# Bergvca/string_grouper

Hardware: AMD Instinct MI355X
Metric: hot-path rows/sec (the device path of match_strings: tokenise + tf-idf + postings + SpGEMM-topn, inputs resident in HBM), 663k-name self-join ntop=10 min_sim=0.8; match_strings end to end: match_strings_rows_per_s (higher is better)
Workload: dtype f32

## Files before the change

### string_grouper_amd/csrc/sg_collapse.hip

```cpp
#include <cstddef>
#include <memory>

#include "sg_internal.h"
#include "sg_scan.h"

template <typename T>
__global__ void __launch_bounds__(256) row_hash_kernel(const int64_t *__restrict__ indptr, const int32_t *__restrict__ indices,
                                                       const T *__restrict__ data, int64_t n_rows, uint64_t *__restrict__ hash,
                                                       uint32_t *__restrict__ row_id ) {
    const int64_t r = ((int64_t)blockIdx.x * blockDim.x + threadIdx.x) >> 4;
    const int sub = threadIdx.x & 15;
    uint64_t h = 0;
    if (r < n_rows) {
        const int64_t lo = indptr[r], hi = indptr[r + 1];
        for (int64_t p = lo + sub; p < hi; p += 16) {
            uint64_t v;
            if (sizeof(T) == 4) v = (uint64_t)__float_as_uint((float)data[p]);
            else v = (uint64_t)__double_as_longlong((double)data[p]);
            uint64_t x = ((uint64_t)(uint32_t)indices[p] << 32) ^ v ^ ((uint64_t)(p - lo) * 0x9E3779B97F4A7C15ull);
            x ^= x >> 33;
            x *= 0xff51afd7ed558ccdull;
            x ^= x >> 33;
            x *= 0xc4ceb9fe1a85ec53ull;
            x ^= x >> 33;
// ... 578 lines not shown
    return SG_OK;
}

struct SortWork {
    uint64_t *hash = nullptr, *hash_sorted = nullptr;
    uint32_t *row_id = nullptr, *row_sorted = nullptr, *head = nullptr, *run_excl = nullptr, *head_pos = nullptr;
    uint32_t *rep_of_row = nullptr, *rank_of_row = nullptr, *is_rep = nullptr, *rep_excl = nullptr, *size = nullptr;
    uint32_t *totals = nullptr;
};

static int sort_and_count(Scratch &scratch, const sg_csr *B, SortWork *w, uint32_t *n_groups) {
    sg_ctx *ctx = scratch.ctx;
    const int64_t n = B->n_rows;
    const unsigned g1 = (unsigned)((n + 255) / 256), g16 = (unsigned)((n * 16 + 255) / 256);
    SG_TRY(scratch.alloc((size_t)n + 1, &w->hash));
    SG_TRY(scratch.alloc((size_t)40, &w->totals));
    SG_TRY(scratch.alloc((size_t)n + 1, &w->hash_sorted));
    SG_TRY(scratch.alloc((size_t)n + 1, &w->row_id));
    SG_TRY(scratch.alloc((size_t)n + 1, &w->row_sorted));
    SG_TRY(scratch.alloc((size_t)n + 1, &w->head));
    SG_TRY(scratch.alloc((size_t)n + 1, &w->run_excl));
    by_dtype(B->dtype, [&](auto tag) {
        using T = decltype(tag);
        hipLaunchKernelGGL(row_hash_kernel<T>, dim3(g16), dim3(256), 0, ctx->stream, B->d_indptr, B->d_indices, (const T *)B->d_data, n,
                           w->hash, w->row_id);
        return SG_OK;
    });
    SG_TRY(sg_sort_pairs_u64_u32(ctx, w->hash, w->row_id, n, w->hash_sorted, w->row_sorted));
    by_dtype(B->dtype, [&](auto tag) {
        using T = decltype(tag);
        hipLaunchKernelGGL(group_heads_kernel<T>, dim3(g1), dim3(256), 0, ctx->stream, B->d_indptr, B->d_indices, (const T *)B->d_data, n,
                           (const uint64_t *)w->hash_sorted, (const uint32_t *)w->row_sorted, w->head);
        return SG_OK;
    });
    SG_TRY(sg_exclusive_scan_u32(ctx, w->head, w->run_excl, n, w->totals));
    SG_HIP_TRY(hipMemcpyAsync(n_groups, w->totals, 4, hipMemcpyDeviceToHost, ctx->stream));
    SG_HIP_TRY(hipStreamSynchronize(ctx->stream));
    return SG_OK;
}

static int sorted_members(Scratch &scratch, int64_t n, SortWork *w, SgCollapse *c) {
    sg_ctx *ctx = scratch.ctx;
    const int64_t n_u = c->n_u;
    const unsigned g1 = (unsigned)((n + 255) / 256);
    SG_TRY(scratch.alloc((size_t)n_u + 1, &w->size));
    SG_TRY(sg_alloc(ctx, (size_t)n + 1, &c->d_gid));
    SG_TRY(sg_alloc(ctx, (size_t)n_u + 2, &c->d_group_ptr));
    SG_TRY(sg_alloc(ctx, (size_t)n + 1, &c->d_members));
    SG_TRY(sg_alloc(ctx, (size_t)n_u + 1, &c->d_rep_rows));
    SG_TRY(scratch.alloc((size_t)n_u + 1, &w->head_pos));
    SG_TRY(scratch.alloc((size_t)n + 1, &w->rep_of_row));
    SG_TRY(scratch.alloc((size_t)n + 1, &w->rank_of_row));
    SG_TRY(scratch.alloc((size_t)n + 1, &w->is_rep));
    SG_TRY(scratch.alloc((size_t)n + 1, &w->rep_excl));
    SG_TRY(SG_ZERO2(ctx, w->is_rep, sizeof(uint32_t) * (size_t)(n + 1), w->size, sizeof(uint32_t) * (size_t)(n_u + 1)));
    hipLaunchKernelGGL(head_pos_kernel, dim3(g1), dim3(256), 0, ctx->stream, (const uint32_t *)w->head, (const uint32_t *)w->run_excl, n,
                       w->head_pos);
    hipLaunchKernelGGL(group_members_kernel, dim3(g1), dim3(256), 0, ctx->stream, (const uint32_t *)w->head,
                       (const uint32_t *)w->run_excl, (const uint32_t *)w->head_pos, (const uint32_t *)w->row_sorted, n, w->rep_of_row,
                       w->rank_of_row, w->is_rep);
    SG_TRY(sg_exclusive_scan_u32(ctx, w->is_rep, w->rep_excl, n, nullptr));
    hipLaunchKernelGGL(group_ids_kernel, dim3(g1), dim3(256), 0, ctx->stream, (const uint32_t *)w->rep_of_row,
                       (const uint32_t *)w->rep_excl, (const uint32_t *)w->is_rep, n, c->d_gid, w->size, c->d_rep_rows,
                       (const int64_t *)nullptr, (int64_t *)nullptr, (int32_t *)nullptr, (unsigned long long *)nullptr);
    SG_TRY(sg_exclusive_scan_u32(ctx, w->size, c->d_group_ptr, n_u, c->d_group_ptr + n_u));
    hipLaunchKernelGGL(group_fill_kernel, dim3(g1), dim3(256), 0, ctx->stream, (const uint32_t *)c->d_gid,
                       (const uint32_t *)w->rank_of_row, (const uint32_t *)c->d_group_ptr, n, c->d_members);
    SG_HIP_TRY(hipGetLastError());
    return SG_OK;
}

static int unique_row_pointers(Scratch &scratch, const sg_csr *B, const SgCollapse *c, int64_t **ptr, int64_t *nnz_u) {
    sg_ctx *ctx = scratch.ctx;
    const int64_t n_u = c->n_u;
    int32_t *len = nullptr;
    SG_TRY(scratch.alloc((size_t)n_u + 1, &len));
    SG_TRY(scratch.alloc((size_t)n_u + 2, ptr));
    hipLaunchKernelGGL(unique_len_kernel, dim3((unsigned)((n_u + 255) / 256)), dim3(256), 0, ctx->stream, B->d_indptr,
                       (const uint32_t *)c->d_rep_rows, n_u, len);
    SG_TRY(sg_exclusive_scan_i32_to_i64(ctx, len, *ptr, n_u));
    SG_HIP_TRY(hipMemcpyAsync(nnz_u, *ptr + n_u, 8, hipMemcpyDeviceToHost, ctx->stream));
    SG_HIP_TRY(hipStreamSynchronize(ctx->stream));
    scratch.keep(*ptr);
    return SG_OK;
}

static int group_by_sort(sg_ctx *ctx, const sg_csr *B, bool forced, bool defer_rows, SgCollapse **out) {
    *out = nullptr;
    const int64_t n = B->n_rows;
    CollapsePtr c;
    int64_t *ptr = nullptr;
    int64_t nnz_u = 0;
    {
        Scratch scratch(ctx);
        SortWork w;
        uint32_t n_groups = 0;
        SG_TRY(sort_and_count(scratch, B, &w, &n_groups));
        if (!worth_grouping(n_groups, n, forced)) return SG_OK;
        c = new_groups(ctx, n);
        if (!c) return SG_ERR_OOM;
        c->n_u = n_groups;
        SG_TRY(sorted_members(scratch, n, &w, c.get()));
        SG_TRY(unique_row_pointers(scratch, B, c.get(), &ptr, &nnz_u));
    }
    SG_TRY(collapse_unique_matrix(ctx, B, c.get(), nnz_u, ptr, defer_rows));
    *out = c.release();
    return SG_OK;
}

int sg_collapse_build(sg_ctx *ctx, const sg_csr *B, SgCollapse **out, bool left_side, bool defer_rows) {
    *out = nullptr;
    bool forced = false;
    if (!wanted(ctx, B, left_side, &forced)) return SG_OK;
    bool by_sort = ctx->opt_is("SG_GROUP_SORT", '1');
    if (!by_sort) SG_TRY(group_by_hash_table(ctx, B, forced, defer_rows, out, &by_sort));
    if (by_sort) SG_TRY(group_by_sort(ctx, B, forced, defer_rows, out));
    return SG_OK;
}

template <typename T>
__global__ void __launch_bounds__(256) expand_simple_kernel(const int32_t *__restrict__ u_cols, const T *__restrict__ u_vals,
                                                            const int32_t *__restrict__ u_cnt, int32_t u_stride,
                                                            const uint32_t *__restrict__ gid ,
                                                            const int32_t *__restrict__ row_list ,
                                                            const uint32_t *__restrict__ group_ptr, const uint32_t *__restrict__ members,
                                                            int64_t n_out, int32_t stride, int32_t *__restrict__ cols,
                                                            T *__restrict__ vals, int32_t *__restrict__ cnt,
                                                            uint32_t *__restrict__ slow_count, uint32_t *__restrict__ slow_rows) {
    const int64_t r = (int64_t)blockIdx.x * blockDim.x + threadIdx.x;
    if (r >= n_out) return;
    const int64_t row = row_list ? (int64_t)row_list[r] : r;
    const int64_t ur = gid ? (int64_t)gid[row] : row;
    const int32_t m = u_cnt[ur];
    const int32_t *uc = u_cols + ur * u_stride;
    const T *uv = u_vals + ur * u_stride;
    int32_t out = 0;
    T prev = (T)0;
    for (int32_t e = 0; e < m && out < stride; ++e) {
        const uint32_t lo = group_ptr[uc[e]], hi = group_ptr[uc[e] + 1];
        const T v = uv[e];
        if (hi - lo != 1u && ((e > 0 && prev == v) || (e + 1 < m && uv[e + 1] == v))) {
            slow_rows[atomicAdd(slow_count, 1u)] = (uint32_t)r;
            return;
        }
        for (uint32_t p = lo; p < hi && out < stride; ++p, ++out) {
            cols[r * stride + out] = (int32_t)members[p];
            vals[r * stride + out] = v;
        }
        prev = v;
    }
    cnt[r] = out;
}

template <typename T>
__global__ void __launch_bounds__(64) expand_merge_kernel(const int32_t *__restrict__ u_cols, const T *__restrict__ u_vals,
                                                          const int32_t *__restrict__ u_cnt, int32_t u_stride,
                                                          const uint32_t *__restrict__ gid, const int32_t *__restrict__ row_list,
                                                          const uint32_t *__restrict__ group_ptr,
                                                          const uint32_t *__restrict__ members, int32_t stride,
                                                          int32_t *__restrict__ cols, T *__restrict__ vals, int32_t *__restrict__ cnt,
                                                          const uint32_t *__restrict__ slow_count, const uint32_t *__restrict__ slow_rows) {
    const int lane = threadIdx.x;
    const uint32_t n_slow = *slow_count;
    for (uint32_t q = blockIdx.x; q < n_slow; q += gridDim.x) {
        const int64_t r = slow_rows[q];
        const int64_t row = row_list ? (int64_t)row_list[r] : r;
        const int64_t ur = gid ? (int64_t)gid[row] : row;
        const int32_t m = u_cnt[ur];
        const int32_t *uc = u_cols + ur * u_stride;
        const T *uv = u_vals + ur * u_stride;
        int32_t out = 0;
        int32_t e0 = 0;
        while (e0 < m && out < stride) {
            const T score = uv[e0];
            int32_t e1 = e0 + 1;
            while (e1 < m && uv[e1] == score) ++e1;
            const int32_t run = e1 - e0;
            if (run <= 64) {
                uint32_t cur = 0, end = 0;
                if (lane < run) {
                    cur = group_ptr[uc[e0 + lane]];
                    end = group_ptr[uc[e0 + lane] + 1];
                }
                uint32_t nxt = (lane < run && cur < end) ? members[cur] : 0xFFFFFFFFu;
                while (out < stride) {
                    uint32_t best = nxt;
#pragma unroll
                    for (int d = 32; d > 0; d >>= 1) best = min(best, (uint32_t)__shfl_xor((int)best, d, 64));
                    if (best == 0xFFFFFFFFu) break;
                    if (lane == 0) {
                        cols[r * stride + out] = (int32_t)best;
                        vals[r * stride + out] = score;
                    }
                    ++out;
                    if (nxt == best) {
                        ++cur;
                        nxt = cur < end ? members[cur] : 0xFFFFFFFFu;
                    }
                }
            } else {
                uint32_t last = 0;
                bool any_written = false;
                while (out < stride) {
                    uint32_t best = 0xFFFFFFFFu;
                    for (int32_t g = lane; g < run; g += 64) {
                        uint32_t lo = group_ptr[uc[e0 + g]], hi = group_ptr[uc[e0 + g] + 1];
                        while (lo < hi) {
                            const uint32_t mid = (lo + hi) >> 1;
                            if (any_written && members[mid] <= last) lo = mid + 1;
                            else hi = mid;
                        }
                        if (lo < group_ptr[uc[e0 + g] + 1]) best = min(best, members[lo]);
                    }
#pragma unroll
                    for (int d = 32; d > 0; d >>= 1) best = min(best, (uint32_t)__shfl_xor((int)best, d, 64));
                    if (best == 0xFFFFFFFFu) break;
                    if (lane == 0) {
                        cols[r * stride + out] = (int32_t)best;
                        vals[r * stride + out] = score;
                    }
                    ++out;
                    last = best;
                    any_written = true;
                }
            }
            e0 = e1;
        }
        if (lane == 0) cnt[r] = out;
    }
}

int sg_collapse_expand(sg_ctx *ctx, const SgCollapse *c, const sg_topn *ru, bool rows_are_groups, sg_topn *out,
                       const int32_t *row_list) {
    const int64_t n_out = out->n_rows;
    if (n_out <= 0) return SG_OK;
    Scratch scratch(ctx);
    uint32_t *slow = nullptr;
    SG_TRY(scratch.alloc((size_t)n_out + 4, &slow));
    SG_TRY(SG_ZERO2(ctx, out->d_counts, sizeof(int32_t) * (size_t)(n_out + 1), slow, 16));
    const unsigned g1 = (unsigned)((n_out + 255) / 256);
    const uint32_t *gid = rows_are_groups ? c->d_gid : nullptr;
    by_dtype(out->dtype, [&](auto tag) {
        using T = decltype(tag);
        hipLaunchKernelGGL(expand_simple_kernel<T>, dim3(g1), dim3(256), 0, ctx->stream, (const int32_t *)ru->d_cols,
                           (const T *)ru->d_vals, (const int32_t *)ru->d_counts, ru->stride, gid, row_list,
                           (const uint32_t *)c->d_group_ptr, (const uint32_t *)c->d_members, n_out, out->stride, out->d_cols,
                           (T *)out->d_vals, out->d_counts, slow, slow + 4);
        hipLaunchKernelGGL(expand_merge_kernel<T>, dim3(2048), dim3(64), 0, ctx->stream, (const int32_t *)ru->d_cols,
                           (const T *)ru->d_vals, (const int32_t *)ru->d_counts, ru->stride, gid, row_list,
                           (const uint32_t *)c->d_group_ptr, (const uint32_t *)c->d_members, out->stride, out->d_cols,
                           (T *)out->d_vals, out->d_counts, (const uint32_t *)slow, (const uint32_t *)(slow + 4));
        return SG_OK;
    });
    SG_HIP_TRY(hipGetLastError());
    return SG_OK;
}
```

### string_grouper_amd/csrc/sg_spgemm_topn.hip

```cpp
#include <cstring>
#include <math.h>

#include <memory>

#include "sg_internal.h"

#include "sg_k4_device.h"
#include "sg_plan.h"

static_assert(SG_PLAN_LANES == SG_TOPN_LANES, "sg_plan.h counts passes and register lists in the kernels' lanes");

typedef float f32x4 __attribute__((ext_vector_type(4)));
typedef double f64x2 __attribute__((ext_vector_type(2)));
template <typename T, typename V>
__device__ __forceinline__ bool any_above(const V &v, T thr);
template <>
__device__ __forceinline__ bool any_above<float, f32x4>(const f32x4 &v, float thr) {
    const uint32_t a = __float_as_uint(v[0]), b = __float_as_uint(v[1]), c = __float_as_uint(v[2]),
                   d = __float_as_uint(v[3]);
    const uint32_t ab = a > b ? a : b, cd = c > d ? c : d;
    return (ab > cd ? ab : cd) > __float_as_uint(thr);
}
template <>
__device__ __forceinline__ bool any_above<double, f64x2>(const f64x2 &v, double thr) {
// ... 559 lines not shown
    a->nnz = A->nnz;
    a->f64 = A->dtype == SG_F64;
    a->is_index_source = built_from(A, Bt);
    b->cosine_like = Bt->cosine_like;
    b->has_filter = Bt->d_filt != nullptr;
    b->tile_form = Bt->tile_form;
    b->pruned_tile = sg_pruned_supports_tile(Bt->tile_log2);
    b->fold_log2 = Bt->fold_log2;
    b->tile_log2 = Bt->tile_log2;
    b->n_tiles = Bt->n_tiles;
    b->n_right = Bt->n_right;
    b->nnz = Bt->nnz;
    b->n_terms = Bt->n_terms;
    const sg_csr *from = companion_source(A, Bt);
    b->source_rows = from ? from->n_rows : -1;
}

static int plan_multiply(sg_ctx *ctx, const sg_csr *A, const sg_postings *Bt, int32_t top_n, double threshold, bool row_range,
                         SgPlan *plan) {
    *plan = SgPlan();
    const SgPlanSwitches sw = multiply_switches(ctx);
    SgPlanCall call;
    call.threshold = plan->threshold = sg_plan_clamp_threshold(threshold);
    call.row_range = row_range;
    plan->index = Bt;
    if (!result_stride(A->n_rows, top_n, Bt->n_right, &plan->stride))
        return row_range ? SG_OK : result_overflow(A->n_rows, plan->stride, "; split the left matrix");
    call.stride = plan->stride;
    SgPlanLeft a;
    SgPlanIndex b;
    describe(A, Bt, &a, &b);

    if (sg_plan_wants_tile_form(a, b, call, sw) && sg_plan_source_fits(b)) {
        SG_TRY(companion(ctx, owner(Bt), SgCompanion::alt_tile, companion_source(A, Bt), &Bt));
        describe(A, Bt, &a, &b);
    }

    bool a_cosine_like = false;
    if (sg_plan_needs_props(a, b, call, sw)) {
        plan->delta = sg_plan_delta(a, b, call, sw);
        float a_n2 = 0.f;
        SG_TRY(sg_csr_props(ctx, A, &a_cosine_like, &a_n2, nullptr));
    }

    plan->form = sg_plan_form(a, b, call, sw, a_cosine_like);

    if (sg_plan_pilot_due(a, b, call, sw, plan->form)) {
        SgPilotPrices prices;
        SG_TRY(sg_csr_ensure_rows(ctx, A));
        SG_TRY(prune_pilot(ctx, A, Bt, a, b, plan->stride, plan->threshold, plan->delta, plan->form == SgPlan::PRUNED_SELFJOIN, &prices));
        plan->form = sg_plan_after_pilot(plan->form, prices, sw);
    }

    const SgOwnIndex own = sg_plan_exact_own_index(a, b, call, sw, plan->form);
    if (own != SgOwnIndex::none) {
        SG_TRY(companion(ctx, owner(Bt), SgCompanion::exact_native, own == SgOwnIndex::from_left ? A : companion_source(A, Bt), &Bt));
        describe(A, Bt, &a, &b);
    }

    plan->index = Bt;
    plan->launch = sg_plan_launch_shape(a, b, plan->stride, ctx->num_cu, ctx->lds_per_cu, sw);
    return SG_OK;
}

static int zero_then_selfjoin_pass(sg_ctx *ctx, const sg_csr *A, const SgPlan &plan, sg_topn *r, uint32_t *counters, size_t n_counters,
                                   size_t n_stat_words, bool *done, int64_t row_lo = 0, int64_t row_hi = -1,
                                   int32_t **d_pairs = nullptr, int64_t *n_pairs = nullptr, int64_t row_step = 1) {
    *done = false;
    SG_TRY(SG_ZERO3(ctx, counters, sizeof(uint32_t) * n_counters, r->d_counts, sizeof(int32_t) * (size_t)A->n_rows,
                    ctx->d_stat_words, n_stat_words * sizeof(int64_t)));
    int st = SG_OK;
    if (sg_plan_selfjoin(plan.form))
        st = sg_spgemm_pruned_symmetric(ctx, A, plan.index, plan.stride, r, plan.threshold, plan.delta,
                                        (unsigned long long *)(ctx->d_stat_words + 2), done, row_lo, row_hi, d_pairs, n_pairs, row_step,
                                        plan.form == SgPlan::EXACT_SELFJOIN);
    ctx->prune_symmetric = *done;
    return st;
}

static int pruned_launches(sg_ctx *ctx, const sg_csr *A, const SgPlan &plan, sg_topn *r, uint32_t *row_counter, uint32_t *handed_count,
                           uint32_t *handed_rows) {
    SgTimer kt(ctx, SG_K_SPGEMM_KERNEL);
    SG_TRY(sg_spgemm_pruned_launch(ctx, A, plan.index, plan.stride < SG_TOPN_LANES ? plan.stride : SG_TOPN_LANES, r, plan.threshold,
                                   plan.delta, row_counter, handed_count, handed_rows, (unsigned long long *)(ctx->d_stat_words + 2)));
    if (plan.stride > SG_TOPN_LANES && A->n_rows > 0) {
        hipLaunchKernelGGL(rows_with_full_lists_kernel, dim3((unsigned)((A->n_rows + 255) / 256)), dim3(256), 0, ctx->stream,
                           (const int32_t *)r->d_counts, A->n_rows, (int32_t)SG_TOPN_LANES, handed_count, handed_rows);
        SG_HIP_TRY(hipGetLastError());
    }
    return SG_OK;
}

static int rows_handed_over(sg_ctx *ctx, const sg_postings *Bt, const uint32_t *handed_count, bool *any) {
    *any = true;
    if (Bt->d_vals != nullptr || Bt->nnz <= 0) return SG_OK;
    uint32_t *h_handed = (uint32_t *)(ctx->h_stat_words + 7);
    *h_handed = 0;
    SG_TRY(sg_fetch(ctx, h_handed, handed_count, 4));
    *any = *h_handed > 0;
    return SG_OK;
}

static int exact_passes(sg_ctx *ctx, const sg_csr *A, const SgPlan &plan, sg_topn *r, uint32_t *counters, const uint32_t *row_list,
                        const uint32_t *row_list_len) {
    const sg_postings *Bt = plan.index;
    const SgLaunchShape &sh = plan.launch;
    if (A->n_rows <= 0) return SG_OK;
    for (int pass = 0, li = 0; pass < sh.n_pass; ++pass) {
        const int pass_off = pass * SG_TOPN_LANES;
        const int keep = plan.stride - pass_off < SG_TOPN_LANES ? plan.stride - pass_off : SG_TOPN_LANES;
        for (int g = 0; g < sh.n_groups; ++g, ++li) {
            const int tb = g * sh.group;
            const int te = tb + sh.group < Bt->n_tiles ? tb + sh.group : Bt->n_tiles;
            SG_TRY(by_dtype(A->dtype, [&](auto tag) {
                using T = decltype(tag);
                return dispatch_spgemm<T>(ctx, A, Bt, tb, te, keep, pass_off, r, (T)plan.threshold, counters + li, sh.grid, row_list, row_list_len);
            }));
        }
    }
    return SG_OK;
}

static int run_plan(sg_ctx *ctx, const sg_csr *A, const SgPlan &plan, sg_topn *r) {
    const sg_postings *Bt = plan.index;
    const bool prune = sg_plan_pruned(plan.form);
    const size_t n_launch = (size_t)plan.launch.n_launch(), n_words = n_launch + 4;
    Scratch tmp(ctx);
    uint32_t *counters = nullptr;
    SG_TRY(tmp.alloc(n_words + (prune ? (size_t)A->n_rows : 0), &counters));
    uint32_t *handed_count = counters + n_launch + 2;
    uint32_t *handed_rows = counters + n_words;

    SgTimer timer(ctx, SG_K_SPGEMM);
    bool selfjoin_done = false;
    SG_TRY(zero_then_selfjoin_pass(ctx, A, plan, r, counters, n_words, 7, &selfjoin_done));
    if (selfjoin_done) return SG_OK;
    SG_TRY(sg_csr_ensure_rows(ctx, A));
    if (!prune) {
        SG_TRY(sg_postings_ensure_full(ctx, Bt));
        SgTimer kt(ctx, SG_K_SPGEMM_KERNEL);
        return exact_passes(ctx, A, plan, r, counters, nullptr, handed_count);
    }
    SG_TRY(pruned_launches(ctx, A, plan, r, counters + n_launch + 1, handed_count, handed_rows));
    bool any_handed = false;
    SG_TRY(rows_handed_over(ctx, Bt, handed_count, &any_handed));
    if (any_handed) {
        SG_TRY(sg_postings_ensure_full(ctx, Bt));
        SG_TRY(exact_passes(ctx, A, plan, r, counters, handed_rows, handed_count));
    }
    SG_HIP_TRY(hipMemcpyAsync(ctx->d_stat_words + 5, handed_count, 4, hipMemcpyDeviceToDevice, ctx->stream));
    return SG_OK;
}

struct InnerMultiply {
    sg_ctx *ctx;
    explicit InnerMultiply(sg_ctx *c) : ctx(c) { ++ctx->inner_multiply_depth; }
    ~InnerMultiply() { --ctx->inner_multiply_depth; }
};

static int spgemm_topn_collapsed(sg_ctx *ctx, const sg_csr *A, const sg_postings *Bt, int32_t top_n, double threshold,
                                 int32_t sort, sg_topn **out) {
    const SgCollapse *c = Bt->collapse;
    int64_t stride64 = top_n;
    if (stride64 > c->n_orig) stride64 = c->n_orig > 0 ? c->n_orig : 1;
    if (stride64 > 2 * SG_TOPN_LANES) {
        const sg_postings *plain = nullptr;
        SG_TRY(companion(ctx, Bt, SgCompanion::plain, &Bt->caller_b_copy, &plain));
        return sg_spgemm_topn(ctx, A, plain, top_n, threshold, sort, out);
    }
    const bool self = built_from(A, Bt);
    sg_postings view = *Bt;
    view.collapse = nullptr;
    view.plain = nullptr;
    view.view_of = Bt;
    sg_topn *groups = nullptr;
    {
        const InnerMultiply inner(ctx);
        SG_TRY(sg_spgemm_topn(ctx, self ? c->unique : A, &view, top_n, threshold, 1, &groups));
    }
    const TopnPtr ru(groups);
    TopnPtr r;
    SG_TRY(topn_alloc(ctx, A->n_rows, c->n_orig, (int32_t)stride64, A->dtype, &r));
    {
        SgTimer timer(ctx, SG_K_ZIP);
        SG_TRY(sg_collapse_expand(ctx, c, ru.get(), self, r.get()));
        if (!sort) SG_TRY(sort_rows_by_column(ctx, r.get()));
        if (A->n_rows > 0 && ctx->inner_multiply_depth == 0) {
            hipLaunchKernelGGL(sum_counts_kernel, dim3(256), dim3(256), 0, ctx->stream, r->d_counts, A->n_rows,
                               (unsigned long long *)(ctx->d_stat_words + 1));
            if (hipGetLastError() != hipSuccess) return SG_ERR_HIP;
        }
    }
    *out = r.release();
    return SG_OK;
}

template <typename T>
__global__ void __launch_bounds__(256) expand_left_rows_kernel(const int32_t *__restrict__ u_cols, const T *__restrict__ u_vals,
                                                               const int32_t *__restrict__ u_cnt, const uint32_t *__restrict__ gid,
                                                               int64_t n_rows, int32_t stride, int32_t *__restrict__ cols,
                                                               T *__restrict__ vals, int32_t *__restrict__ cnt) {
    const int64_t cell = (int64_t)blockIdx.x * blockDim.x + threadIdx.x;
    if (cell >= n_rows * stride) return;
    const int64_t r = cell / stride;
    const int32_t e = (int32_t)(cell - r * stride);
    const int64_t g = gid[r];
    const int32_t m = u_cnt[g];
    if (e == 0) cnt[r] = m;
    if (e < m) {
        cols[cell] = u_cols[g * stride + e];
        vals[cell] = u_vals[g * stride + e];
    }
}

static int spgemm_topn_left_groups(sg_ctx *ctx, const sg_csr *A, const sg_postings *Bt, int32_t top_n, double threshold, int32_t sort,
                                   sg_topn **out, bool *done) {
    *done = false;
    if (A->left_state == 1) return SG_OK;
    if (A->left_state == 0) {
        SgCollapse *g = nullptr;
        bool cl = false;
        float n2 = 0.f;
        SG_TRY(sg_csr_props(ctx, A, &cl, &n2));
        if (cl) SG_TRY(sg_collapse_build(ctx, A, &g, true));
        A->left_groups = g;
        A->left_state = g ? 2 : 1;
        if (!g) return SG_OK;
    }
    const SgCollapse *g = A->left_groups;
    sg_topn *groups = nullptr;
    g->unique->left_state = 1;
    {
        const InnerMultiply inner(ctx);
        SG_TRY(sg_spgemm_topn(ctx, g->unique, Bt, top_n, threshold, sort, &groups));
    }
    const TopnPtr ru(groups);
    TopnPtr r;
    SG_TRY(topn_alloc(ctx, A->n_rows, ru->n_cols, ru->stride, ru->dtype, &r));
    if (A->n_rows > 0) {
        SgTimer timer(ctx, SG_K_ZIP);
        const int64_t cells = A->n_rows * (int64_t)ru->stride;
        const unsigned grid = (unsigned)((cells + 255) / 256);
        by_dtype(ru->dtype, [&](auto tag) {
            using T = decltype(tag);
            hipLaunchKernelGGL(expand_left_rows_kernel<T>, dim3(grid), dim3(256), 0, ctx->stream, (const int32_t *)ru->d_cols,
                               (const T *)ru->d_vals, (const int32_t *)ru->d_counts, (const uint32_t *)g->d_gid, A->n_rows,
                               ru->stride, r->d_cols, (T *)r->d_vals, r->d_counts);
            return SG_OK;
        });
        hipLaunchKernelGGL(sum_counts_kernel, dim3(256), dim3(256), 0, ctx->stream, r->d_counts, A->n_rows,
                           (unsigned long long *)(ctx->d_stat_words + 1));
        if (hipGetLastError() != hipSuccess) return SG_ERR_HIP;
    }
    *out = r.release();
    *done = true;
    return SG_OK;
}

static int left_groups_apply(sg_ctx *ctx, const sg_csr *A, const sg_postings *Bt, int32_t top_n, bool *apply) {
    *apply = false;
    const bool off = ctx->opt_is("SG_COLLAPSE", '0') || ctx->opt_is("SG_COLLAPSE_LEFT", '0');
    if (off && A->left_groups) {
        sg_collapse_free(A->left_groups);
        A->left_groups = nullptr;
        A->left_state = 0;
    }
    if (built_from(A, Bt) || off || A->left_state == 1 || A->n_cols != Bt->n_terms || A->dtype != Bt->dtype || top_n < 1) return SG_OK;
    int32_t stride = 0;
    if (!result_stride(A->n_rows, top_n, Bt->collapse ? Bt->collapse->n_orig : Bt->n_right, &stride))
        return result_overflow(A->n_rows, stride, "; split the left matrix");
    *apply = true;
    return SG_OK;
}

extern "C" int sg_spgemm_topn(sg_ctx *ctx, const sg_csr *A, const sg_postings *Bt, int32_t top_n, double threshold,
                              int32_t sort, sg_topn **out) {
    SG_REQUIRE(ctx && A && Bt && out, "null argument");
    bool group_left = false;
    SG_TRY(left_groups_apply(ctx, A, Bt, top_n, &group_left));
    if (group_left) {
        bool done = false;
        SG_TRY(spgemm_topn_left_groups(ctx, A, Bt, top_n, threshold, sort, out, &done));
        if (done) return SG_OK;
    }
    if (Bt->collapse) {
        SG_REQUIRE(A->n_cols == Bt->n_terms && A->dtype == Bt->dtype && top_n >= 1, "A and B differ in columns or value type, or top_n < 1");
        return spgemm_topn_collapsed(ctx, A, Bt, top_n, threshold, sort, out);
    }
    SG_REQUIRE(A->n_cols == Bt->n_terms, "A and B have different numbers of columns (vocabulary size)");
    SG_REQUIRE(A->dtype == Bt->dtype, "A and B have different value types");
    SG_REQUIRE(top_n >= 1, "top_n must be >= 1");
    SgPlan plan;
    SG_TRY(plan_multiply(ctx, A, Bt, top_n, threshold, false, &plan));
    Bt = plan.index;
    TopnPtr r;
    SG_TRY(topn_alloc(ctx, A->n_rows, Bt->n_right, plan.stride, A->dtype, &r));
    SG_TRY(run_plan(ctx, A, plan, r.get()));
    if (!sort) SG_TRY(sort_rows_by_column(ctx, r.get()));
    if (A->nnz > 0 && built_from(A, Bt))
        hipLaunchKernelGGL(count_macs_selfjoin_kernel, dim3(64), dim3(256), 0, ctx->stream, (const uint32_t *)Bt->d_term_len,
                           Bt->n_terms, (unsigned long long *)ctx->d_stat_words);
    else if (A->nnz > 0)
        hipLaunchKernelGGL(count_macs_kernel, dim3(512), dim3(256), 0, ctx->stream, A->d_indptr, A->d_indices,
                           A->n_rows, (const uint32_t *)Bt->d_term_len, (unsigned long long *)ctx->d_stat_words);
    if (A->n_rows > 0 && ctx->inner_multiply_depth == 0)
        hipLaunchKernelGGL(sum_counts_kernel, dim3(256), dim3(256), 0, ctx->stream, r->d_counts, A->n_rows,
                           (unsigned long long *)(ctx->d_stat_words + 1));
    record_bytes(ctx, A, Bt, plan.threshold);
    if (hipGetLastError() != hipSuccess) return SG_ERR_HIP;
    *out = r.release();
    return SG_OK;
}

extern "C" int sg_selfjoin_range(sg_ctx *ctx, const sg_csr *A, const sg_postings *Bt, int32_t top_n, double threshold,
                                 int64_t row_lo, int64_t row_hi, sg_topn **out, int32_t **d_pairs, int64_t *n_pairs,
                                 int32_t *pair_words, int32_t *applicable, int64_t row_step) {
    if (row_step < 1) row_step = 1;
    SG_REQUIRE(ctx && A && Bt && out && d_pairs && n_pairs && pair_words && applicable, "null argument");
    SG_REQUIRE(A->n_cols == Bt->n_terms && A->dtype == Bt->dtype, "A and B differ in columns or value type");
    SG_REQUIRE(top_n >= 1, "top_n must be >= 1");
    SG_REQUIRE(row_lo >= 0 && row_lo <= row_hi && row_hi <= A->n_rows, "row range outside the matrix");
    *out = nullptr;
    *d_pairs = nullptr;
    *n_pairs = 0;
    *pair_words = A->dtype == SG_F64 ? 4 : 3;
    *applicable = 0;
    if (Bt->collapse) {
        const SgCollapse *c = Bt->collapse;
        if (!built_from(A, Bt)) return SG_OK;
        if (row_hi > c->n_u) {
            sg_set_error("row range [%lld, %lld) outside the %lld groups of the index (sg_postings_rows)", (long long)row_lo,
                         (long long)row_hi, (long long)c->n_u);
            return SG_ERR_BADARG;
        }
        sg_postings view = *Bt;
        view.collapse = nullptr;
        view.plain = nullptr;
        const int st_u = sg_selfjoin_range(ctx, c->unique, &view, top_n, threshold, row_lo, row_hi, out, d_pairs, n_pairs, pair_words,
                                           applicable, row_step);
        if (st_u == SG_OK && *out) (*out)->top_n_asked = top_n;
// ... 191 lines not shown
```

Measured before the change: 111.6 million.

## Expand collapsed top-n rows with DPP sub-wave kernel and fused count sum

Replaces the one-thread-per-row expansion of collapsed group results with a kernel that assigns a 4/8/16-lane sub-wave to each row. It uses DPP row moves for tie detection and for prefix sums of group sizes, so members are scattered in parallel, and it processes several rows per thread to raise memory-level parallelism. The kernel and the merge kernel also accumulate the total result count, which removes the separate sum_counts launch. The grid becomes persistent, capped at twice the CU count. The new paths add complexity, a device-side atomic per block, and an optional probe path that synchronises the stream.

Result: no change. 111.1 million (-0.4%).

```diff
diff --git a/string_grouper_amd/csrc/sg_collapse.hip b/string_grouper_amd/csrc/sg_collapse.hip
--- a/string_grouper_amd/csrc/sg_collapse.hip
+++ b/string_grouper_amd/csrc/sg_collapse.hip
@@ -754,6 +754,163 @@
     cnt[r] = out;
 }
 
+template <int CTRL>
+__device__ __forceinline__ uint32_t row_move(uint32_t x) {
+    return (uint32_t)__builtin_amdgcn_update_dpp(0, (int)x, CTRL, 0xf, 0xf, true);
+}
+template <int CTRL>
+__device__ __forceinline__ float row_move(float x) {
+    return __uint_as_float(row_move<CTRL>(__float_as_uint(x)));
+}
+template <int CTRL>
+__device__ __forceinline__ double row_move(double x) {
+    const uint64_t b = (uint64_t)__double_as_longlong(x);
+    const uint64_t m = ((uint64_t)row_move<CTRL>((uint32_t)(b >> 32)) << 32) | row_move<CTRL>((uint32_t)b);
+    return __longlong_as_double((long long)m);
+}
+
+template <typename T, int W>
+__device__ __forceinline__ void subwave_trip(int sl, int first, int32_t e, int32_t m, T v, T below_edge, T above_edge, uint32_t lo,
+                                             uint32_t hi, uint32_t out, int32_t stride, uint32_t &at, uint32_t &n, uint32_t &total,
+                                             bool &queued) {
+    const bool has = e < m;
+    const uint32_t size = hi - lo;
+    T below = row_move<0x111>(v), above = row_move<0x101>(v);
+    if (sl == 0) below = below_edge;
+    if (sl == W - 1) above = above_edge;
+    const bool tie = has && size != 1u && ((e > 0 && below == v) || (e + 1 < m && above == v));
+    uint32_t incl = size, t;
+    t = row_move<0x111>(incl); if (sl >= 1) incl += t;
+    t = row_move<0x112>(incl); if (sl >= 2) incl += t;
+    if (W >= 8) { t = row_move<0x114>(incl); if (sl >= 4) incl += t; }
+    if (W >= 16) { t = row_move<0x118>(incl); if (sl >= 8) incl += t; }
+    total = size;
+    total += row_move<0xB1>(total);
+    total += row_move<0x4E>(total);
+    if (W >= 8) total += row_move<0x141>(total);
+    if (W >= 16) total += row_move<0x140>(total);
+    at = out + (incl - size);
+    const unsigned long long ties = __ballot(tie && at < (uint32_t)stride);
+    queued = ((ties >> first) & ((1ull << W) - 1ull)) != 0;
+    n = 0;
+    if (has && !queued && at < (uint32_t)stride) n = size < (uint32_t)stride - at ? size : (uint32_t)stride - at;
+}
+
+#define SG_EXPAND_BLOCK 512
+template <typename T, int W, int R>
+__global__ void __launch_bounds__(SG_EXPAND_BLOCK) expand_subwave_kernel(const int32_t *__restrict__ u_cols, const T *__restrict__ u_vals,
+                                                             const int32_t *__restrict__ u_cnt, int32_t u_stride,
+                                                             const uint32_t *__restrict__ gid, const int32_t *__restrict__ row_list,
+                                                             const uint32_t *__restrict__ group_ptr, const uint32_t *__restrict__ members,
+                                                             int64_t n_out, int32_t stride, int32_t *__restrict__ cols,
+                                                             T *__restrict__ vals, int32_t *__restrict__ cnt,
+                                                             uint32_t *__restrict__ slow_count, uint32_t *__restrict__ slow_rows,
+                                                             unsigned long long *__restrict__ sum_out) {
+    static_assert(W == 4 || W == 8 || W == 16, "a sub-wave is a quad, half a DPP row or a whole one");
+    const int sl = threadIdx.x & (W - 1);
+    const int first = threadIdx.x & 63 & ~(W - 1);
+    const int64_t n_sub = (int64_t)gridDim.x * blockDim.x / W;
+    uint32_t written = 0;
+    for (int64_t r0 = ((int64_t)blockIdx.x * blockDim.x + threadIdx.x) / W; r0 < n_out; r0 += n_sub * R) {
+        int64_t ur[R];
+        int32_t m[R], g[R];
+        T v[R], v_edge[R];
+        uint32_t lo[R], hi[R], at[R], n[R], out[R], member0[R];
+        bool queued[R];
+#pragma unroll
+        for (int k = 0; k < R; ++k) {
+            const int64_t r = r0 + k * n_sub;
+            ur[k] = -1;
+            if (r < n_out) {
+                const int64_t row = row_list ? (int64_t)row_list[r] : r;
+                ur[k] = gid ? (int64_t)gid[row] : row;
+            }
+        }
+#pragma unroll
+        for (int k = 0; k < R; ++k) {
+            m[k] = 0, g[k] = 0, v[k] = (T)0, v_edge[k] = (T)0;
+            if (ur[k] >= 0) {
+                m[k] = u_cnt[ur[k]];
+                if (sl < u_stride) g[k] = u_cols[ur[k] * u_stride + sl], v[k] = u_vals[ur[k] * u_stride + sl];
+                if (sl == W - 1 && W < u_stride) v_edge[k] = u_vals[ur[k] * u_stride + W];
+            }
+        }
+#pragma unroll
+        for (int k = 0; k < R; ++k) {
+            lo[k] = hi[k] = 0;
+            if (sl < m[k]) lo[k] = group_ptr[g[k]], hi[k] = group_ptr[g[k] + 1];
+        }
+#pragma unroll
+        for (int k = 0; k < R; ++k) {
+            subwave_trip<T, W>(sl, first, sl, m[k], v[k], (T)0, v_edge[k], lo[k], hi[k], 0u, stride, at[k], n[k], out[k], queued[k]);
+            member0[k] = n[k] ? members[lo[k]] : 0u;
+        }
+#pragma unroll
+        for (int k = 0; k < R; ++k) {
+            const int64_t r = r0 + k * n_sub;
+            if (n[k]) {
+                cols[r * stride + at[k]] = (int32_t)member0[k];
+                vals[r * stride + at[k]] = v[k];
+                for (uint32_t j = 1; j < n[k]; ++j) {
+                    cols[r * stride + at[k] + j] = (int32_t)members[lo[k] + j];
+                    vals[r * stride + at[k] + j] = v[k];
+                }
+            }
+        }
+#pragma unroll
+        for (int k = 0; k < R; ++k) {
+            if (ur[k] < 0) continue;
+            const int64_t r = r0 + k * n_sub;
+            const int32_t *uc = u_cols + ur[k] * u_stride;
+            const T *uv = u_vals + ur[k] * u_stride;
+            uint32_t o = out[k];
+            bool q = queued[k];
+            for (int32_t base = W; !q && base < m[k] && o < (uint32_t)stride; base += W) {
+                const int32_t e = base + sl;
+                const bool has = e < m[k];
+                const int32_t ge = has ? uc[e] : 0;
+                const T ve = has ? uv[e] : (T)0;
+                const T below_edge = (has && sl == 0) ? uv[e - 1] : (T)0;
+                const T above_edge = (sl == W - 1 && e + 1 < m[k]) ? uv[e + 1] : (T)0;
+                uint32_t l = 0, h = 0, a, c, total;
+                if (has) l = group_ptr[ge], h = group_ptr[ge + 1];
+                subwave_trip<T, W>(sl, first, e, m[k], ve, below_edge, above_edge, l, h, o, stride, a, c, total, q);
+                for (uint32_t j = 0; j < c; ++j) {
+                    cols[r * stride + a + j] = (int32_t)members[l + j];
+                    vals[r * stride + a + j] = ve;
+                }
+                o += total;
+            }
+            if (o > (uint32_t)stride) o = (uint32_t)stride;
+            if (sl == 0) {
+                if (q) {
+                    slow_rows[atomicAdd(slow_count, 1u)] = (uint32_t)r;
+                } else {
+                    cnt[r] = (int32_t)o;
+                    written += o;
+                }
+            }
+        }
+    }
+    if (sum_out) {
+        __shared__ uint32_t wave_sum[SG_EXPAND_BLOCK / 64];
+        uint32_t s = written;
+        s += row_move<0xB1>(s);
+        s += row_move<0x4E>(s);
+        s += row_move<0x141>(s);
+        s += row_move<0x140>(s);
+        const uint32_t wave = (uint32_t)__builtin_amdgcn_readlane((int)s, 0) + (uint32_t)__builtin_amdgcn_readlane((int)s, 16) +
+                              (uint32_t)__builtin_amdgcn_readlane((int)s, 32) + (uint32_t)__builtin_amdgcn_readlane((int)s, 48);
+        if ((threadIdx.x & 63) == 0) wave_sum[threadIdx.x >> 6] = wave;
+        __syncthreads();
+        if (threadIdx.x == 0) {
+            unsigned long long block = 0;
+            for (unsigned w = 0; w < blockDim.x / 64; ++w) block += wave_sum[w];
+            if (block) atomicAdd(sum_out, block);
+        }
+    }
+}
+
 template <typename T>
 __global__ void __launch_bounds__(64) expand_merge_kernel(const int32_t *__restrict__ u_cols, const T *__restrict__ u_vals,
                                                           const int32_t *__restrict__ u_cnt, int32_t u_stride,
@@ -761,7 +918,8 @@
                                                           const uint32_t *__restrict__ group_ptr,
                                                           const uint32_t *__restrict__ members, int32_t stride,
                                                           int32_t *__restrict__ cols, T *__restrict__ vals, int32_t *__restrict__ cnt,
-                                                          const uint32_t *__restrict__ slow_count, const uint32_t *__restrict__ slow_rows) {
+                                                          const uint32_t *__restrict__ slow_count, const uint32_t *__restrict__ slow_rows,
+                                                          unsigned long long *__restrict__ sum_out ) {
     const int lane = threadIdx.x;
     const uint32_t n_slow = *slow_count;
     for (uint32_t q = blockIdx.x; q < n_slow; q += gridDim.x) {
@@ -828,32 +986,62 @@
             }
             e0 = e1;
         }
-        if (lane == 0) cnt[r] = out;
-    }
-}
-
-int sg_collapse_expand(sg_ctx *ctx, const SgCollapse *c, const sg_topn *ru, bool rows_are_groups, sg_topn *out,
-                       const int32_t *row_list) {
+        if (lane == 0) {
+            cnt[r] = out;
+            if (sum_out && out) atomicAdd(sum_out, (unsigned long long)out);
+        }
+    }
+}
+
+int sg_collapse_expand_counted(sg_ctx *ctx, const SgCollapse *c, const sg_topn *ru, bool rows_are_groups, sg_topn *out,
+                               const int32_t *row_list, unsigned long long *sum_out, bool *summed) {
+    if (summed) *summed = false;
     const int64_t n_out = out->n_rows;
     if (n_out <= 0) return SG_OK;
     Scratch scratch(ctx);
     uint32_t *slow = nullptr;
     SG_TRY(scratch.alloc((size_t)n_out + 4, &slow));
     SG_TRY(SG_ZERO2(ctx, out->d_counts, sizeof(int32_t) * (size_t)(n_out + 1), slow, 16));
-    const unsigned g1 = (unsigned)((n_out + 255) / 256);
+    int lanes = ctx->opt_int("SG_EXPAND_LANES", 4);
+    if (lanes != 16 && lanes != 8 && lanes != 4) lanes = 1;
+    if (lanes > 1 && ru->stride > 16 * lanes) lanes = 1;
+    if (!summed) sum_out = nullptr;
+    if (lanes == 1) sum_out = nullptr;
     const uint32_t *gid = rows_are_groups ? c->d_gid : nullptr;
     by_dtype(out->dtype, [&](auto tag) {
         using T = decltype(tag);
-        hipLaunchKernelGGL(expand_simple_kernel<T>, dim3(g1), dim3(256), 0, ctx->stream, (const int32_t *)ru->d_cols,
-                           (const T *)ru->d_vals, (const int32_t *)ru->d_counts, ru->stride, gid, row_list,
-                           (const uint32_t *)c->d_group_ptr, (const uint32_t *)c->d_members, n_out, out->stride, out->d_cols,
-                           (T *)out->d_vals, out->d_counts, slow, slow + 4);
+        const auto launch = [&](auto kern, int64_t block, int64_t rows_per_block, int64_t most_blocks, auto... tail) {
+            int64_t grid = (n_out + rows_per_block - 1) / rows_per_block;
+            if (most_blocks > 0 && grid > most_blocks) grid = most_blocks;
+            hipLaunchKernelGGL(kern, dim3((unsigned)grid), dim3((unsigned)block), 0, ctx->stream,
+                               (const int32_t *)ru->d_cols, (const T *)ru->d_vals, (const int32_t *)ru->d_counts, ru->stride, gid,
+                               row_list, (const uint32_t *)c->d_group_ptr, (const uint32_t *)c->d_members, n_out, out->stride,
+                               out->d_cols, (T *)out->d_vals, out->d_counts, slow, slow + 4, tail...);
+        };
+        const int64_t most = (int64_t)ctx->num_cu * 2;
+        if (lanes == 4) launch(expand_subwave_kernel<T, 4, 4>, SG_EXPAND_BLOCK, SG_EXPAND_BLOCK / 4 * 4, most, sum_out);
+        else if (lanes == 8) launch(expand_subwave_kernel<T, 8, 4>, SG_EXPAND_BLOCK, SG_EXPAND_BLOCK / 8 * 4, most, sum_out);
+        else if (lanes == 16) launch(expand_subwave_kernel<T, 16, 4>, SG_EXPAND_BLOCK, SG_EXPAND_BLOCK / 16 * 4, most, sum_out);
+        else launch(expand_simple_kernel<T>, 256, 256, 0);
         hipLaunchKernelGGL(expand_merge_kernel<T>, dim3(2048), dim3(64), 0, ctx->stream, (const int32_t *)ru->d_cols,
                            (const T *)ru->d_vals, (const int32_t *)ru->d_counts, ru->stride, gid, row_list,
                            (const uint32_t *)c->d_group_ptr, (const uint32_t *)c->d_members, out->stride, out->d_cols,
-                           (T *)out->d_vals, out->d_counts, (const uint32_t *)slow, (const uint32_t *)(slow + 4));
+                           (T *)out->d_vals, out->d_counts, (const uint32_t *)slow, (const uint32_t *)(slow + 4), sum_out);
         return SG_OK;
     });
     SG_HIP_TRY(hipGetLastError());
-    return SG_OK;
-}
+    if (summed) *summed = sum_out != nullptr;
+    if (ctx->opt_is("SG_EXPAND_PROBE", '1')) {
+        SG_HIP_TRY(hipMemcpyAsync(ctx->h_fetch, slow, 4, hipMemcpyDeviceToHost, ctx->stream));
+        SG_HIP_TRY(hipStreamSynchronize(ctx->stream));
+        const std::string queued = std::to_string(ctx->h_fetch[0]);
+        std::lock_guard<std::mutex> g(ctx->mu);
+        ctx->opts["SG_EXPAND_QUEUED"] = queued;
+    }
+    return SG_OK;
+}
+
+int sg_collapse_expand(sg_ctx *ctx, const SgCollapse *c, const sg_topn *ru, bool rows_are_groups, sg_topn *out,
+                       const int32_t *row_list) {
+    return sg_collapse_expand_counted(ctx, c, ru, rows_are_groups, out, row_list, nullptr, nullptr);
+}
diff --git a/string_grouper_amd/csrc/sg_spgemm_topn.hip b/string_grouper_amd/csrc/sg_spgemm_topn.hip
--- a/string_grouper_amd/csrc/sg_spgemm_topn.hip
+++ b/string_grouper_amd/csrc/sg_spgemm_topn.hip
@@ -735,6 +735,9 @@
     return SG_OK;
 }
 
+int sg_collapse_expand_counted(sg_ctx *ctx, const SgCollapse *c, const sg_topn *ru, bool rows_are_groups, sg_topn *out,
+                               const int32_t *row_list, unsigned long long *sum_out, bool *summed);
+
 struct InnerMultiply {
     sg_ctx *ctx;
     explicit InnerMultiply(sg_ctx *c) : ctx(c) { ++ctx->inner_multiply_depth; }
@@ -766,9 +769,12 @@
     SG_TRY(topn_alloc(ctx, A->n_rows, c->n_orig, (int32_t)stride64, A->dtype, &r));
     {
         SgTimer timer(ctx, SG_K_ZIP);
-        SG_TRY(sg_collapse_expand(ctx, c, ru.get(), self, r.get()));
+        const bool count = A->n_rows > 0 && ctx->inner_multiply_depth == 0;
+        bool counted = false;
+        SG_TRY(sg_collapse_expand_counted(ctx, c, ru.get(), self, r.get(), nullptr,
+                                          count ? (unsigned long long *)(ctx->d_stat_words + 1) : nullptr, &counted));
         if (!sort) SG_TRY(sort_rows_by_column(ctx, r.get()));
-        if (A->n_rows > 0 && ctx->inner_multiply_depth == 0) {
+        if (count && !counted) {
             hipLaunchKernelGGL(sum_counts_kernel, dim3(256), dim3(256), 0, ctx->stream, r->d_counts, A->n_rows,
                                (unsigned long long *)(ctx->d_stat_words + 1));
             if (hipGetLastError() != hipSuccess) return SG_ERR_HIP;
```
